# oxfordcontrol/COSMO.jl

Measured on AMD Instinct MI355X. Metric: ADMM iterations/sec (fp64) at fixed (n,m,nnz,cone), higher is better.
Workload: dtype f64

## Files before the change

cosmo.jl_amd/csrc/psd_polar.hip:

```cpp
#include "psd_internal.h"
#include "polar_tiles.h"
#include <math.h>
#include <stdlib.h>
#include <string.h>
#include <algorithm>
#include <mutex>

#define PK 16
#ifndef POLAR_PREFETCH_DEPTH
#define POLAR_PREFETCH_DEPTH 2
#endif
#define PLD 80
static_assert(PK == kPolarPanelK, "the planner's k panel");
static_assert(sizeof(QTile) == sizeof(int4), "the quadrant list is uploaded as the kernels' int4 array");

struct SkSync { unsigned ticket; unsigned timeout; unsigned pad[14]; unsigned flag[1]; };
struct PolarDev {
  int gate;
  int rounds;
  int verified;
  int unverified;
  int projections;
  int pad[3];
  real err_last, err_max;
};

static const real kPolarLift[3] = {3.8438259784376458, -2.5414431444903771, 0.42553478492344637};
#define POLAR_NFIN 5
static const real kPolarFinish[POLAR_NFIN][3] = {
    {3.4931704678738202, -2.370790022242379, 0.42240833954524776},
    {2.7077959763108326, -2.015093165601975, 0.45683257965863566},
    {1.9693651031668091, -1.3512768962961363, 0.3852630352029357},
    {1.875, -1.25, 0.375},
    {1.875, -1.25, 0.375}};
#define POLAR_RLIFT 3
#define POLAR_NFIN_LARGE (REAL_IS_FLOAT ? 4 : POLAR_NFIN)
#define POLAR_RLIFT_LARGE (REAL_IS_FLOAT ? 4 : POLAR_RLIFT)

#define POLAR_LIFT_CAP 18
struct PolarPlan {
  std::vector<PolarCone> cones;
  real* W = nullptr;
  real* parts = nullptr;
  real* nrm = nullptr;
  int k_lift = REAL_IS_FLOAT ? 5 : 9;
  bool klift_forced = false;
  int max_rounds = 2;
  int rescale = 1;
  int batch_occ = 3;
  real tol_factor = 8.0;
  PolarDev* dev = nullptr;
  PolarDev seen;
  long long launches[4] = {0, 0, 0, 0};
  int streamk = 0;
  real* sk_scratch = nullptr;
  SkSync* sk_sync = nullptr;
  int sk_gmax = 0;
  unsigned sk_base = 0, sk_epoch = 0;
  int products_last_large = 0, products_last_batch = 0;
  std::vector<BatchCone> bcones;
  BatchCone* d_bcones = nullptr;
  int4* d_btiles = nullptr;
  int nbtiles = 0, nbtiles96 = 0;
  int speculate = 0;
  int* gate_host = nullptr;
  int batch_wave = 0;
  int batch_ragged = 1;
  void* d_rtiles = nullptr;
  int nrtiles = 0;
  int dataflow = 0;
  void* d_df_tiles = nullptr;
  int* d_df_cone_nt = nullptr;
  unsigned* d_df_sync = nullptr;
  int df_xoff[9] = {0, 0, 0, 0, 0, 0, 0, 0, 0};
  int df_grid = 0;
  int df_pair = 3;
  int df_ntiles = 0;
  long long df_launches = 0, df_timed = 0;
  int df_nprod = 0;
  double df_seconds = 0.0;
  hipEvent_t df_ev[2] = {nullptr, nullptr};
  int df_ev_pending = 0;
  void* h_rtiles = nullptr;
  void* rep_host = nullptr;
  void* d_rtiles_rep = nullptr;
  int nrep = 0;
  long long repair_launch_tiles = 0, repair_trains = 0;
  double batch_flops_performed = 0.0, batch_flops_useful = 0.0;
  int batch_ts96 = 0;
  real* BW = nullptr;
  real* bparts = nullptr;
  real* bnrm = nullptr;
  int* bgate = nullptr;
  int adapt = 0;
  int compact_repair = 1;
  std::vector<LiftDepth> bdepth;
  int* d_lgate = nullptr;
  int* d_ubuf = nullptr;
  int* bgate_host = nullptr;
  int lgate_kmax = -1;
  long long depth_fail = 0, depth_down = 0, depth_proj = 0;
  int seen_proj_batch = 0;
  std::vector<LiftDepth> ldepth;
  int seen_proj_large = 0;
  double wprod_last = 0.0;
  bool adaptive() const { return adapt && !speculate && !klift_forced && k_lift <= POLAR_LIFT_CAP; }
};

extern "C" int32_t cosmo_hip_polar_schedule(int32_t k_lift, double* abc, int32_t* nsteps) {
  if (k_lift < 0 || k_lift > 64 || !nsteps) return COSMO_HIP_ERR_INVALID;
  *nsteps = k_lift + POLAR_NFIN;
  if (!abc) return COSMO_HIP_OK;
  for (int t = 0; t < k_lift; ++t) for (int q = 0; q < 3; ++q) abc[3 * t + q] = (double)kPolarLift[q];
  for (int t = 0; t < POLAR_NFIN; ++t) for (int q = 0; q < 3; ++q) abc[3 * (k_lift + t) + q] = (double)kPolarFinish[t][q];
  return COSMO_HIP_OK;
}

namespace {

__device__ __forceinline__ long long svec_index(int i, int j) { return (long long)j * (j + 1) / 2 + i; }


__device__ __forceinline__ real polar_read(const real* __restrict__ x, int kind, int d, int i, int j) {
  const real isq2 = 0.70710678118654752440;
  if (kind == COSMO_HIP_PSD_TRIANGLE) {
    const int a = i < j ? i : j, b = i < j ? j : i;
    const real t = x[svec_index(a, b)];
    return (a == b) ? t : isq2 * t;
  }
  if (kind == COSMO_HIP_PSD_SQUARE) {
    const int a = i < j ? i : j, b = i < j ? j : i;
    return (x[(long long)b * d + a] + x[(long long)a * d + b]) / R(2.0);
  }
  const int r = d / 2;
  const int bi = i >= r, bj = j >= r, ii = i - bi * r, jj = j - bj * r;
  const int a = ii < jj ? ii : jj, b = ii < jj ? jj : ii;
  if (bi == bj) { const real t = x[svec_index(a, b)]; return (a == b) ? t : isq2 * t; }
  if (ii == jj) return 0.0;
  real im = isq2 * x[(long long)r * (r + 1) / 2 + (long long)b * (b - 1) / 2 + a];
  if (ii > jj) im = -im;
  return (bi == 1) ? im : -im;
}
__device__ __forceinline__ void polar_write(real* __restrict__ x, int kind, int d, int i, int j, real v) {
  const real sq2 = 1.41421356237309504880;
  if (kind == COSMO_HIP_PSD_TRIANGLE) { x[svec_index(i, j)] = (i == j) ? v : sq2 * v; return; }
  if (kind == COSMO_HIP_PSD_SQUARE) { x[(long long)j * d + i] = v; x[(long long)i * d + j] = v; return; }
  const int r = d / 2;
  if (j < r) { x[svec_index(i, j)] = (i == j) ? v : sq2 * v; return; }
  if (i < r) { const int jj = j - r; if (i < jj) x[(long long)r * (r + 1) / 2 + (long long)jj * (jj - 1) / 2 + i] = sq2 * (-v); }
}

__global__ __launch_bounds__(COSMO_BS) void k_polar_populate(const Ctl* __restrict__ ctl, int guard, PolarCone cn, const real* __restrict__ s,
                                                             real* __restrict__ X, real* __restrict__ parts) {
  if (guard && ctl->halt) return;
  __shared__ real red[COSMO_BS / 64];
  const real* x = s + cn.off;
  const int d = cn.d, ld = cn.ld;
  real acc = 0.0;
  for (int j = blockIdx.x; j < ld; j += gridDim.x) {
    for (int i = threadIdx.x; i < ld; i += COSMO_BS) {
      real v = 0.0;
      if (i < d && j < d) { v = polar_read(x, cn.kind, d, i, j); acc += v * v; }
      X[(long long)j * ld + i] = v;
    }
  }
  acc = block_sum(acc, red);
  if (threadIdx.x == 0) parts[blockIdx.x] = acc;
}

__global__ __launch_bounds__(COSMO_BS) void k_polar_scale(const Ctl* __restrict__ ctl, int guard, long long n, int nparts, const real* __restrict__ parts,
                                                          const real* __restrict__ X, real* __restrict__ U, real* __restrict__ nrm_out) {
  if (guard && ctl->halt) return;
  __shared__ real red[COSMO_BS / 64];
  const real nf = sqrt(reduce_partials_sum(parts, nparts, red));
  const real inv = (nf > R(0.0)) ? R(2.0) / nf : R(0.0);
  if (blockIdx.x == 0 && threadIdx.x == 0) *nrm_out = nf;
// ... 1030 lines not shown

#define BPX 16
__global__ __launch_bounds__(COSMO_BS) void k_bpolar_populate(const Ctl* __restrict__ ctl, int guard, const BatchCone* __restrict__ cones,
                                                              const real* __restrict__ s, real* __restrict__ W, real* __restrict__ parts) {
  if (guard && ctl->halt) return;
  __shared__ real red[COSMO_BS / 64];
  const BatchCone cn = cones[blockIdx.y];
  const real* x = s + cn.off;
  real* X = W + cn.woff;
  const int d = cn.d, ld = cn.ld;
  real acc = 0.0;
  for (int j = blockIdx.x; j < ld; j += gridDim.x) {
    for (int i = threadIdx.x; i < ld; i += COSMO_BS) {
      real v = 0.0;
      if (i < d && j < d) { v = polar_read(x, cn.kind, d, i, j); acc += v * v; }
      X[(long long)j * ld + i] = v;
    }
  }
  acc = block_sum(acc, red);
  if (threadIdx.x == 0) parts[(size_t)blockIdx.y * 2 * BPX + blockIdx.x] = acc;
}
__global__ __launch_bounds__(COSMO_BS) void k_bpolar_scale(const Ctl* __restrict__ ctl, int guard, const BatchCone* __restrict__ cones,
                                                           const real* __restrict__ parts, real* __restrict__ W, real* __restrict__ bnrm,
                                                           const int* __restrict__ ubuf) {
  if (guard && ctl->halt) return;
  const BatchCone cn = cones[blockIdx.y];
  real nf2 = 0.0;
  for (int k = 0; k < BPX; ++k) nf2 += parts[(size_t)blockIdx.y * 2 * BPX + k];
  const real nf = sqrt(nf2);
  const real inv = (nf > R(0.0)) ? R(2.0) / nf : R(0.0);
  if (blockIdx.x == 0 && threadIdx.x == 0) bnrm[blockIdx.y] = nf;
  const long long n2 = (long long)cn.ld * cn.ld;
  const real* X = W + cn.woff;
  real* U = W + cn.woff + (ubuf ? ubuf[blockIdx.y] : 1) * n2;
  for (long long i = (long long)blockIdx.x * COSMO_BS + threadIdx.x; i < n2; i += (long long)gridDim.x * COSMO_BS) U[i] = X[i] * inv;
}
__global__ __launch_bounds__(COSMO_BS) void k_bpolar_finish(const Ctl* __restrict__ ctl, int guard, const BatchCone* __restrict__ cones,
                                                            real* __restrict__ W, int iu, real* __restrict__ s, real* __restrict__ parts) {
  if (guard && ctl->halt) return;
  __shared__ real red[COSMO_BS / 64];
  const BatchCone cn = cones[blockIdx.y];
  const long long n2 = (long long)cn.ld * cn.ld;
  const real* X = W + cn.woff;
  const real* U = W + cn.woff + iu * n2;
  const real* H = W + cn.woff + 3 * n2;
  real* x = s + cn.off;
  const int d = cn.d, ld = cn.ld;
  real tr = 0.0;
  for (int j = blockIdx.x; j < d; j += gridDim.x) {
    for (int i = threadIdx.x; i <= j; i += COSMO_BS) {
      const long long o = (long long)j * ld + i;
      const real v = (X[o] + H[o]) / R(2.0);
      polar_write(x, cn.kind, d, i, j, v);
      const real u = U[o];
      tr += (i == j) ? (u + u * u) : R(2.0) * u * u;
    }
  }
  tr = block_sum(tr, red);
  if (threadIdx.x == 0) parts[(size_t)blockIdx.y * 2 * BPX + BPX + blockIdx.x] = tr;
}
__global__ void k_bpolar_rank(const Ctl* __restrict__ ctl, int guard, int n, const BatchCone* __restrict__ cones, const real* __restrict__ parts,
                              int* __restrict__ rank) {
  if (guard && ctl->halt) return;
  const int c = blockIdx.x * blockDim.x + threadIdx.x;
  if (c >= n) return;
  real tr = 0.0;
  for (int k = 0; k < BPX; ++k) tr += parts[(size_t)c * 2 * BPX + BPX + k];
  rank[cones[c].idx] = (int)llround(tr / (cones[c].kind == COSMO_HIP_PSD_TRIANGLE_COMPLEX ? R(4.0) : R(2.0)));
}

__global__ __launch_bounds__(COSMO_BS) void k_bpolar_sumsq(const Ctl* __restrict__ ctl, int guard, const int* __restrict__ gate, const BatchCone* __restrict__ cones,
                                                           const real* __restrict__ W, int ig, real* __restrict__ vparts) {
  if (guard && ctl->halt) return;
  if (gate && !gate[blockIdx.y]) return;
  __shared__ real red[COSMO_BS / 64];
  const BatchCone cn = cones[blockIdx.y];
  const long long n2 = (long long)cn.ld * cn.ld;
  const real* G = W + cn.woff + ig * n2;
  real acc = 0.0;
  for (long long i = (long long)blockIdx.x * COSMO_BS + threadIdx.x; i < n2; i += (long long)gridDim.x * COSMO_BS) { const real v = G[i]; acc += v * v; }
  acc = block_sum(acc, red);
  if (threadIdx.x == 0) vparts[(size_t)blockIdx.y * BPX + blockIdx.x] = acc;
}
__global__ __launch_bounds__(COSMO_BS) void k_bpolar_decide(const Ctl* __restrict__ ctl, int guard, PolarDev* __restrict__ pd, int* __restrict__ bgate, int round,
                                                            int last, int n, const BatchCone* __restrict__ cones, const real* __restrict__ vparts,
                                                            const real* __restrict__ bnrm, real tol_factor) {
  if (guard && ctl->halt) return;
  if (round > 0 && !pd->gate) return;
  __shared__ real red[COSMO_BS / 64];
  real emax = 0.0, nfail = 0.0, nchk = 0.0;
  for (int c = threadIdx.x; c < n; c += COSMO_BS) {
    if (round > 0 && !bgate[c]) continue;
    real g2 = 0.0;
    for (int k = 0; k < BPX; ++k) g2 += vparts[(size_t)c * BPX + k];
    const real nf = bnrm[c];
    const real err = (nf > R(0.0)) ? R(0.5) * sqrt(g2) / nf : R(0.0);
    const bool ok = !(err > tol_factor * cones[c].d * PSD_EPS);
    bgate[c] = (!ok && !last) ? 1 : 0;
    nchk += 1.0;
    if (!ok) nfail += 1.0;
    emax = (err > emax || err != err) ? err : emax;
  }
  emax = block_max(emax, red);
  nfail = block_sum(nfail, red);
  nchk = block_sum(nchk, red);
  if (threadIdx.x != 0) return;
  pd->err_last = emax;
  if (emax > pd->err_max || emax != emax) pd->err_max = emax;
  if (round == 0) pd->projections += 1; else pd->rounds += 1;
  if (nfail == R(0.0)) { pd->verified += 1; pd->gate = 0; }
  else if (last) { pd->unverified += 1; pd->gate = 0; }
  else pd->gate = 1;
  (void)nchk;
}

}

void polar_plan_destroy(cosmo_hip_handle* h) {
  PolarPlan* q = static_cast<PolarPlan*>(h->psd_polar);
  if (!q) return;
  if (q->W) (void)hipFree(q->W);
  if (q->parts) (void)hipFree(q->parts);
  if (q->nrm) (void)hipFree(q->nrm);
  if (q->gate_host) (void)hipHostFree(q->gate_host);
  if (q->sk_scratch) (void)hipFree(q->sk_scratch);
  if (q->sk_sync) (void)hipFree(q->sk_sync);
  if (q->d_bcones) (void)hipFree(q->d_bcones);
  if (q->d_btiles) (void)hipFree(q->d_btiles);
  if (q->d_rtiles) (void)hipFree(q->d_rtiles);
  if (q->d_rtiles_rep) (void)hipFree(q->d_rtiles_rep);
  if (q->rep_host) (void)hipHostFree(q->rep_host);
  free(q->h_rtiles);
  if (q->BW) (void)hipFree(q->BW);
  if (q->bparts) (void)hipFree(q->bparts);
  if (q->bnrm) (void)hipFree(q->bnrm);
  if (q->bgate) (void)hipFree(q->bgate);
  if (q->d_lgate) (void)hipFree(q->d_lgate);
  if (q->d_ubuf) (void)hipFree(q->d_ubuf);
  if (q->bgate_host) (void)hipHostFree(q->bgate_host);
  if (q->d_df_tiles) (void)hipFree(q->d_df_tiles);
  if (q->d_df_cone_nt) (void)hipFree(q->d_df_cone_nt);
  if (q->d_df_sync) (void)hipFree(q->d_df_sync);
  if (q->df_ev[0]) { (void)hipEventDestroy(q->df_ev[0]); (void)hipEventDestroy(q->df_ev[1]); }
  if (q->dev) (void)hipFree(q->dev);
  delete q;
  h->psd_polar = nullptr;
}

bool polar_enabled(const cosmo_hip_handle* h) { return h->psd_polar != nullptr; }

struct PolarKnobs {
  int large_jacobi = -1, k_lift = -1, adapt = 0, compact_repair = 1, rescale = 1, speculate = -1, rounds = -1, patience = 3;
  int streamk = 0, ts = 0, sk = 0;
  long long skg = 0;
  int ts96 = 0, wave = 0, flat = 0, ragged = 1, paired = -1, sort = 1, dataflow = -1, dataflow_grid = -1, occ = -1;
};

static PolarKnobs polar_read_knobs() {
  PolarKnobs k;
  auto flag = [](const char* name, int dflt) { const char* e = getenv(name); return e ? (atoi(e) ? 1 : 0) : dflt; };
  auto within = [](const char* name, int lo, int hi, int dflt) { const char* e = getenv(name); const int v = e ? atoi(e) : dflt; return (v >= lo && v <= hi) ? v : dflt; };
  if (const char* e = getenv("COSMO_HIP_PSD_LARGE")) k.large_jacobi = (e[0] == 'j') ? 1 : 0;
  if (const char* e = getenv("COSMO_HIP_POLAR_KLIFT")) k.k_lift = std::min(40, std::max(0, atoi(e)));
  k.adapt = flag("COSMO_HIP_POLAR_ADAPT", k.adapt);
  if (const char* e = getenv("COSMO_HIP_POLAR_PATIENCE")) k.patience = std::max(1, atoi(e));
  k.compact_repair = flag("COSMO_HIP_POLAR_COMPACT_REPAIR", k.compact_repair);
  k.rescale = flag("COSMO_HIP_POLAR_RESCALE", k.rescale);
  k.speculate = flag("COSMO_HIP_POLAR_SPECULATE", k.speculate);
  if (const char* e = getenv("COSMO_HIP_POLAR_ROUNDS")) k.rounds = std::min(8, std::max(0, atoi(e)));
  k.streamk = flag("COSMO_HIP_POLAR_STREAMK", k.streamk);
  if (const char* e = getenv("COSMO_HIP_POLAR_TS")) k.ts = atoi(e);
  if (const char* e = getenv("COSMO_HIP_POLAR_SK")) k.sk = atoi(e);
  if (const char* e = getenv("COSMO_HIP_POLAR_SKG")) k.skg = atoll(e);
  k.ts96 = flag("COSMO_HIP_POLAR_BATCH_TS96", k.ts96);
  k.wave = flag("COSMO_HIP_POLAR_BATCH_WAVE", k.wave);
  k.flat = getenv("COSMO_HIP_POLAR_BATCH_FLAT") ? 1 : 0;
  k.ragged = flag("COSMO_HIP_POLAR_BATCH_RAGGED", k.ragged);
  k.sort = flag("COSMO_HIP_POLAR_BATCH_SORT", k.sort);
  k.occ = within("COSMO_HIP_POLAR_BATCH_OCC", 3, 4, k.occ);
  k.paired = within("COSMO_HIP_POLAR_PAIRED", 0, 3, k.paired);
  k.dataflow = flag("COSMO_HIP_POLAR_DATAFLOW", k.dataflow);
  k.dataflow_grid = within("COSMO_HIP_POLAR_DATAFLOW_GRID", 8, 8192, k.dataflow_grid);
  return k;
}

static void polar_set_func_attributes(const PolarPlan* q) {
  if (q->bcones.empty()) return;
  if (q->batch_ragged) {
    (void)hipFuncSetAttribute((const void*)k_polar_dataflow<4>, hipFuncAttributeMaxDynamicSharedMemorySize, GemmCfg<64>::SMEM);
    (void)hipFuncSetAttribute((const void*)k_polar_dataflow_pair<4>, hipFuncAttributeMaxDynamicSharedMemorySize, DF_PAIR_SMEM);
    (void)hipFuncSetAttribute((const void*)k_symm_gemm_batch_r<0, 3>, hipFuncAttributeMaxDynamicSharedMemorySize, GemmCfg<64>::SMEM);
    (void)hipFuncSetAttribute((const void*)k_symm_gemm_batch_r<1, 3>, hipFuncAttributeMaxDynamicSharedMemorySize, GemmCfg<64>::SMEM);
    (void)hipFuncSetAttribute((const void*)k_symm_gemm_batch_r<0, 4>, hipFuncAttributeMaxDynamicSharedMemorySize, GemmCfg<64>::SMEM);
    (void)hipFuncSetAttribute((const void*)k_symm_gemm_batch_r<1, 4>, hipFuncAttributeMaxDynamicSharedMemorySize, GemmCfg<64>::SMEM);
  }
  (void)hipFuncSetAttribute((const void*)k_symm_gemm_batch<0, 3, 64>, hipFuncAttributeMaxDynamicSharedMemorySize, GemmCfg<64>::SMEM);
  (void)hipFuncSetAttribute((const void*)k_symm_gemm_batch<1, 3, 64>, hipFuncAttributeMaxDynamicSharedMemorySize, GemmCfg<64>::SMEM);
  (void)hipFuncSetAttribute((const void*)k_symm_gemm_batch<0, 4, 64>, hipFuncAttributeMaxDynamicSharedMemorySize, GemmCfg<64>::SMEM);
  (void)hipFuncSetAttribute((const void*)k_symm_gemm_batch<1, 4, 64>, hipFuncAttributeMaxDynamicSharedMemorySize, GemmCfg<64>::SMEM);
  (void)hipFuncSetAttribute((const void*)k_symm_gemm_batch<0, 2, 96>, hipFuncAttributeMaxDynamicSharedMemorySize, GemmCfg<96>::SMEM);
  (void)hipFuncSetAttribute((const void*)k_symm_gemm_batch<1, 2, 96>, hipFuncAttributeMaxDynamicSharedMemorySize, GemmCfg<96>::SMEM);
}

template <class T>
static int32_t polar_upload(cosmo_hip_handle* h, T** dst, const void* src, size_t bytes) {
  HIPCHK(h, hipMalloc((void**)dst, bytes));
  HIPCHK(h, hipMemcpy(*dst, src, bytes, hipMemcpyHostToDevice));
  return COSMO_HIP_OK;
}

int32_t polar_plan_create(cosmo_hip_handle* h) {
  polar_plan_destroy(h);
  PsdPlan* p = h->psd;
  if (!p) return COSMO_HIP_OK;
  const PolarKnobs k = polar_read_knobs();
  std::vector<int> large_list, batch_list = p->polar_batch;
  const bool jac = k.large_jacobi >= 0 ? k.large_jacobi == 1 : h->psd_mode == 1;
  if (!jac) large_list = p->large;
  p->large_by_polar = !jac;
  for (int idx : p->cplx) { if (p->cones[idx].d > 256) large_list.push_back(idx); else batch_list.push_back(idx); }
  if (large_list.empty() && batch_list.empty()) return COSMO_HIP_OK;
  PolarPlan* q = new PolarPlan();
  h->psd_polar = q;
  q->klift_forced = k.k_lift >= 0;
  if (q->klift_forced) q->k_lift = k.k_lift;
  q->adapt = k.adapt; q->compact_repair = k.compact_repair; q->rescale = k.rescale; q->streamk = k.streamk;
  q->batch_ts96 = k.ts96; q->batch_wave = k.wave;
  q->speculate = k.speculate >= 0 ? k.speculate : (large_list.size() > 2 ? 1 : 0);
  if (k.rounds >= 0) q->max_rounds = k.rounds;
  q->batch_ragged = (k.ragged && !k.ts96 && !k.wave) ? 1 : 0;
  if (k.paired >= 0) q->df_pair = k.paired;
  PolarTileOpts o;
  o.ts96 = k.ts96; o.flat = k.flat; o.ragged = q->batch_ragged; o.pair = q->df_pair; o.sort = k.sort;
  o.streamk = k.streamk; o.ts = k.ts; o.sk = k.sk; o.skg = k.skg;
  HIPCHK(h, hipHostMalloc((void**)&q->gate_host, 8 * sizeof(int), hipHostMallocDefault));
  for (int i = 0; i < 8; ++i) q->gate_host[i] = 0;
  HIPCHK(h, hipMalloc((void**)&q->dev, sizeof(PolarDev)));
  HIPCHK(h, hipMemset(q->dev, 0, sizeof(PolarDev)));
  memset(&q->seen, 0, sizeof(PolarDev));
  if (!large_list.empty()) {
    long long woff = 0;
    for (int idx : large_list) {
      const PsdConeDev& c = p->cones[idx];
      PolarCone pc;
      pc.idx = idx; pc.off = c.off; pc.d = c.d; pc.kind = c.kind;
      polar_plan_large(o, pc);
      q->sk_gmax = std::max(q->sk_gmax, pc.skg);
      pc.woff = woff;
      woff += 4LL * pc.ld * pc.ld;
      q->cones.push_back(pc);
    }
    HIPCHK(h, hipMalloc((void**)&q->W, sizeof(real) * (size_t)woff));
    HIPCHK(h, hipMalloc((void**)&q->parts, sizeof(real) * 2 * COSMO_MAX_PARTIALS * q->cones.size()));
    HIPCHK(h, hipMalloc((void**)&q->nrm, sizeof(real) * q->cones.size()));
    if (q->sk_gmax > 0) {
      const size_t slot = (size_t)SKG_TS * SKG_TS;
      HIPCHK(h, hipMalloc((void**)&q->sk_scratch, sizeof(real) * slot * (size_t)q->sk_gmax));
      const size_t sb = sizeof(SkSync) + sizeof(unsigned) * (size_t)q->sk_gmax;
      HIPCHK(h, hipMalloc((void**)&q->sk_sync, sb));
      HIPCHK(h, hipMemset(q->sk_sync, 0, sb));
    }
  }
  if (!batch_list.empty()) {
    std::vector<PolarBatchIn> in;
    for (int idx : batch_list) { const PsdConeDev& c = p->cones[idx]; in.push_back(PolarBatchIn{c.d, c.off, c.kind, idx}); }
    PolarBatchPlan bp;
    if (const char* err = polar_plan_batch(in, o, bp)) return cosmo_fail(h, COSMO_HIP_ERR_INVALID, err);
    const size_t nb = bp.cones.size();
    q->bcones = bp.cones;
    q->nbtiles = bp.nbtiles; q->nbtiles96 = bp.nbtiles96;
    q->batch_flops_performed = bp.flops_performed; q->batch_flops_useful = bp.flops_useful;
    if (q->batch_ragged) {
      q->nrtiles = (int)bp.rtiles.size();
      q->df_ntiles = bp.df_ntiles;
      for (int x = 0; x <= kPolarXcds; ++x) q->df_xoff[x] = bp.xoff[x];
      if (q->df_pair) CHK(polar_upload(h, &q->d_df_tiles, bp.pairs.data(), sizeof(RPair) * bp.pairs.size()));
      else CHK(polar_upload(h, &q->d_df_tiles, bp.items.data(), sizeof(RTile) * bp.items.size()));
      CHK(polar_upload(h, &q->d_df_cone_nt, bp.cone_nt.data(), sizeof(int) * nb));
      HIPCHK(h, hipMalloc((void**)&q->d_df_sync, sizeof(unsigned) * (DF_SYNC_DONE + nb)));
      hipDeviceProp_t prop;
      HIPCHK(h, hipGetDeviceProperties(&prop, h->device));
      const int slots = std::max(1, prop.multiProcessorCount) * (q->df_pair ? 2 : 4);
      q->df_grid = k.dataflow_grid >= 0 ? k.dataflow_grid : std::max(1, prop.multiProcessorCount) * 4;
      int nmin = INT32_MAX;
      for (int x = 0; x < kPolarXcds; ++x) nmin = std::min(nmin, q->df_xoff[x + 1] - q->df_xoff[x]);
      q->dataflow = k.dataflow >= 0 ? k.dataflow : (nmin >= slots / kPolarXcds ? 1 : 0);
      const size_t rbytes = sizeof(RTile) * bp.rtiles.size();
      CHK(polar_upload(h, &q->d_rtiles, bp.rtiles.data(), rbytes));
      q->h_rtiles = malloc(rbytes);
      if (!q->h_rtiles) return cosmo_fail(h, COSMO_HIP_ERR_HIP, "out of host memory");
      memcpy(q->h_rtiles, bp.rtiles.data(), rbytes);
      HIPCHK(h, hipMalloc((void**)&q->d_rtiles_rep, rbytes));
      HIPCHK(h, hipHostMalloc((void**)&q->rep_host, rbytes));
    }
    HIPCHK(h, hipMalloc((void**)&q->BW, sizeof(real) * (size_t)bp.work));
    HIPCHK(h, hipMemset(q->BW, 0, sizeof(real) * (size_t)bp.work));
    CHK(polar_upload(h, &q->d_bcones, q->bcones.data(), sizeof(BatchCone) * nb));
    CHK(polar_upload(h, &q->d_btiles, bp.qtiles.data(), sizeof(QTile) * bp.qtiles.size()));
    HIPCHK(h, hipMalloc((void**)&q->bparts, sizeof(real) * 3 * BPX * nb));
    HIPCHK(h, hipMalloc((void**)&q->bnrm, sizeof(real) * nb));
    HIPCHK(h, hipMalloc((void**)&q->bgate, sizeof(int) * nb));
    HIPCHK(h, hipMemset(q->bgate, 0, sizeof(int) * nb));
    q->bdepth.assign(nb, LiftDepth{q->k_lift, 0, k.patience});
    HIPCHK(h, hipMalloc((void**)&q->d_lgate, sizeof(int) * nb * POLAR_LIFT_CAP));
    HIPCHK(h, hipMalloc((void**)&q->d_ubuf, sizeof(int) * nb));
    HIPCHK(h, hipHostMalloc((void**)&q->bgate_host, sizeof(int) * nb, hipHostMallocDefault));
    q->lgate_kmax = -1;
    q->batch_occ = k.occ >= 0 ? k.occ : (q->batch_ragged ? 4 : 3);
  }
  polar_set_func_attributes(q);
  return COSMO_HIP_OK;
}

bool polar_has_batch(const cosmo_hip_handle* h) { const PolarPlan* q = static_cast<const PolarPlan*>(h->psd_polar); return q && !q->bcones.empty(); }
bool polar_has_large(const cosmo_hip_handle* h) { const PolarPlan* q = static_cast<const PolarPlan*>(h->psd_polar); return q && !q->cones.empty(); }

template <int EPI>
static void launch_bgemm(PolarPlan* q, hipStream_t st, const Ctl* ctl, int guard, const int* gate, int ia, int ib, int icin, int ic, real alpha, real beta) {
  auto ragged = [&](int ntiles, const void* tiles) {
    const auto kern = q->batch_occ == 4 ? k_symm_gemm_batch_r<EPI, 4> : k_symm_gemm_batch_r<EPI, 3>;
    hipLaunchKernelGGL(kern, dim3(ntiles), dim3(256), GemmCfg<64>::SMEM, st, ctl, guard, gate, (const RTile*)tiles, q->d_bcones, q->BW, ia, ib, icin, ic, alpha, beta);
  };
  if (q->batch_ragged && q->nrep > 0) {
    ragged(q->nrep, q->d_rtiles_rep);
    q->repair_launch_tiles += q->nrep;
    return;
  }
  if (q->batch_ragged && q->nrtiles > 0) {
    ragged(q->nrtiles, q->d_rtiles);
    return;
  }
  if (q->nbtiles96 > 0)
    hipLaunchKernelGGL((k_symm_gemm_batch<EPI, 2, 96>), dim3(q->nbtiles96), dim3(256), GemmCfg<96>::SMEM, st, ctl, guard, gate, q->d_btiles + q->nbtiles,
                       q->d_bcones, q->BW, ia, ib, icin, ic, alpha, beta);
  if (q->nbtiles > 0 && q->batch_wave) {
    hipLaunchKernelGGL((k_symm_gemm_batch_w<EPI>), dim3(q->nbtiles), dim3(64), 0, st, ctl, guard, gate, q->d_btiles, q->d_bcones, q->BW, ia, ib, icin, ic, alpha, beta);
  } else if (q->nbtiles > 0) {
    const auto kern = q->batch_occ == 4 ? k_symm_gemm_batch<EPI, 4, 64> : k_symm_gemm_batch<EPI, 3, 64>;
    hipLaunchKernelGGL(kern, dim3(q->nbtiles), dim3(256), GemmCfg<64>::SMEM, st, ctl, guard, gate, q->d_btiles, q->d_bcones, q->BW, ia, ib, icin, ic, alpha, beta);
  }
}

int32_t polar_enqueue_project_batch(cosmo_hip_handle* h, real* s, int guard) {
  PolarPlan* q = static_cast<PolarPlan*>(h->psd_polar);
  PsdPlan* p = h->psd;
  hipStream_t st = h->stream;
  const int n = (int)q->bcones.size();
  real* vparts = q->bparts + (size_t)2 * BPX * n;
  const bool adapt = q->adaptive();
  int kmax = q->k_lift;
  if (adapt) {
    kmax = 0;
    for (int c = 0; c < n; ++c) kmax = std::max(kmax, q->bdepth[c].k);
    if (q->lgate_kmax != kmax) {
      std::vector<int> lg((size_t)std::max(kmax, 1) * n, 0), ub((size_t)n, 1);
      for (int c = 0; c < n; ++c) {
        const int t0 = kmax - q->bdepth[c].k;
        for (int t = t0; t < kmax; ++t) lg[(size_t)t * n + c] = 1;
        ub[(size_t)c] = (t0 & 1) ? 2 : 1;
      }
      HIPCHK(h, hipMemcpyAsync(q->d_lgate, lg.data(), sizeof(int) * lg.size(), hipMemcpyHostToDevice, st));
      HIPCHK(h, hipMemcpyAsync(q->d_ubuf, ub.data(), sizeof(int) * ub.size(), hipMemcpyHostToDevice, st));
      HIPCHK(h, hipStreamSynchronize(st));
      q->lgate_kmax = kmax;
    }
  }
  hipLaunchKernelGGL(k_bpolar_populate, dim3(BPX, n), dim3(COSMO_BS), 0, st, h->ctl, guard, q->d_bcones, s, q->BW, q->bparts);
  hipLaunchKernelGGL(k_bpolar_scale, dim3(BPX, n), dim3(COSMO_BS), 0, st, h->ctl, guard, q->d_bcones, q->bparts, q->BW, q->bnrm, adapt ? (const int*)q->d_ubuf : (const int*)nullptr);
  int iu = 1, iy = 2, products = 0;
  DfArgs dfa;
  bool df = q->dataflow && q->batch_ragged && q->nrtiles > 0 && !adapt && !h->profiling && 3 * (kmax + POLAR_NFIN) + 2 <= DF_MAX_PROD;
  dfa.nprod = 0;
  auto product = [&](int epi, const int* gate, int ia, int ib, int icin, int ic, real alpha, real beta) {
    if (df) { DfProd& pr = dfa.prod[dfa.nprod++]; pr.ia = ia; pr.ib = ib; pr.icin = icin; pr.ic = ic; pr.epi = epi; pr.pad = 0; pr.alpha = alpha; pr.beta = beta; return; }
    if (epi) launch_bgemm<1>(q, st, h->ctl, guard, gate, ia, ib, icin, ic, alpha, beta);
    else launch_bgemm<0>(q, st, h->ctl, guard, gate, ia, ib, icin, ic, alpha, beta);
  };
  auto flush_dataflow = [&]() -> int32_t {
    if (!df) return COSMO_HIP_OK;
    for (int x = 0; x < 9; ++x) dfa.xoff[x] = q->df_xoff[x];
    HIPCHK(h, hipMemsetAsync(q->d_df_sync, 0, sizeof(unsigned) * (DF_SYNC_DONE + q->bcones.size()), st));
    if (!q->df_ev[0]) { HIPCHK(h, hipEventCreate(&q->df_ev[0])); HIPCHK(h, hipEventCreate(&q->df_ev[1])); }
    if (q->df_ev_pending && hipEventQuery(q->df_ev[1]) == hipSuccess) {
      float ms = 0.f;
      if (hipEventElapsedTime(&ms, q->df_ev[0], q->df_ev[1]) == hipSuccess) { q->df_seconds += 1e-3 * (double)ms; q->df_timed += 1; }
      q->df_ev_pending = 0;
    }
    (void)hipGetLastError();
    const bool timed = !q->df_ev_pending;
    if (timed) HIPCHK(h, hipEventRecord(q->df_ev[0], st));
    if (q->df_pair)
      hipLaunchKernelGGL((k_polar_dataflow_pair<4>), dim3(q->df_grid), dim3(512), DF_PAIR_SMEM, st, h->ctl, guard, (const RPair*)q->d_df_tiles, (const int*)q->d_df_cone_nt,
                         q->d_df_sync, q->BW, dfa);
    else
      hipLaunchKernelGGL((k_polar_dataflow<4>), dim3(q->df_grid), dim3(256), GemmCfg<64>::SMEM, st, h->ctl, guard, (const RTile*)q->d_df_tiles, (const int*)q->d_df_cone_nt,
                         q->d_df_sync, q->BW, dfa);
    if (timed) { HIPCHK(h, hipEventRecord(q->df_ev[1], st)); q->df_ev_pending = 1; }
    q->df_launches += 1; q->df_nprod = dfa.nprod;
    df = false;
    return COSMO_HIP_OK;
  };
  auto step = [&](const real* co, const int* gate) {
    product(0, gate, iu, iu, iu, iy, 1.0, 0.0);
    product(1, gate, iy, iy, iy, 3, co[2], co[1]);
    product(1, gate, iu, 3, iu, iy, 1.0, co[0]);
    std::swap(iu, iy);
    products += 3; q->launches[3] += 3;
  };
  auto verify = [&](int round, const int* gate) -> int32_t {
    product(0, gate, iu, 0, 0, 3, 1.0, 0.0);
    product(1, gate, iu, 3, 0, iy, 1.0, -1.0);
    CHK(flush_dataflow());
    hipLaunchKernelGGL(k_bpolar_sumsq, dim3(BPX, n), dim3(COSMO_BS), 0, st, h->ctl, guard, gate, q->d_bcones, q->BW, iy, vparts);
    hipLaunchKernelGGL(k_bpolar_decide, dim3(1), dim3(COSMO_BS), 0, st, h->ctl, guard, q->dev, q->bgate, round, round == q->max_rounds ? 1 : 0, n, q->d_bcones,
                       vparts, q->bnrm, q->tol_factor);
    products += 2; q->launches[3] += 2;
    return COSMO_HIP_OK;
  };
  for (int t = 0; t < kmax; ++t) step(kPolarLift, adapt ? (const int*)(q->d_lgate + (size_t)t * n) : (const int*)nullptr);
  for (int t = 0; t < POLAR_NFIN; ++t) step(kPolarFinish[t], nullptr);
  CHK(verify(0, nullptr));
  q->products_last_batch = products;
  { double wsum = 0.0, w3 = 0.0;
    for (int c = 0; c < n; ++c) { const double d3 = (double)q->bcones[c].d * q->bcones[c].d * q->bcones[c].d; w3 += d3; wsum += d3 * (3.0 * ((adapt ? q->bdepth[c].k : kmax) + POLAR_NFIN) + 2.0); }
    q->wprod_last = w3 > 0.0 ? wsum / w3 : 0.0; }
  for (int r = 1; r <= q->max_rounds; ++r) {
    if (!q->speculate) {
      HIPCHK(h, hipMemcpyAsync(q->gate_host, &q->dev->gate, (adapt && r == 1 ? 5 : 1) * sizeof(int), hipMemcpyDeviceToHost, st));
      if (r == 1 && q->bgate_host) HIPCHK(h, hipMemcpyAsync(q->bgate_host, q->bgate, sizeof(int) * (size_t)n, hipMemcpyDeviceToHost, st));
      HIPCHK(h, hipStreamSynchronize(st));
      if (adapt && r == 1 && q->gate_host[4] != q->seen_proj_batch) {
        q->seen_proj_batch = q->gate_host[4];
        q->depth_proj += 1;
        bool changed = false;
        for (int c = 0; c < n; ++c) {
          if (*q->gate_host && q->bgate_host[c]) { q->depth_fail += 1; if (q->bdepth[c].fail(POLAR_LIFT_CAP)) changed = true; }
          else if (q->bdepth[c].pass(0)) { q->depth_down += 1; changed = true; }
        }
        if (changed) q->lgate_kmax = -1;
      }
      if (!*q->gate_host) break;
    }
    int rlift = POLAR_RLIFT;
    if (q->compact_repair && q->batch_ragged && q->h_rtiles && q->bgate_host && !q->speculate) {
      if (r == 1) {
        const RTile* all = (const RTile*)q->h_rtiles; RTile* dst = (RTile*)q->rep_host;
        int cnt = 0;
        for (int t = 0; t < q->nrtiles; ++t) if (all[t].cone >= 0 && q->bgate_host[all[t].cone]) dst[cnt++] = all[t];
        if (cnt > 0) {
          HIPCHK(h, hipMemcpyAsync(q->d_rtiles_rep, dst, sizeof(RTile) * (size_t)cnt, hipMemcpyHostToDevice, st));
          q->nrep = cnt; q->repair_trains += 1;
        }
        if (adapt) rlift = 1;
      }
    }
    for (int t = 0; t < rlift; ++t) step(kPolarLift, q->bgate);
    for (int t = 0; t < POLAR_NFIN; ++t) step(kPolarFinish[t], q->bgate);
    CHK(verify(r, q->bgate));
  }
  q->nrep = 0;
  hipLaunchKernelGGL(k_bpolar_finish, dim3(BPX, n), dim3(COSMO_BS), 0, st, h->ctl, guard, q->d_bcones, q->BW, iu, s, q->bparts);
  hipLaunchKernelGGL(k_bpolar_rank, dim3((n + 63) / 64), dim3(64), 0, st, h->ctl, guard, n, q->d_bcones, q->bparts, p->rank);
  HIPCHK(h, hipGetLastError());
  return COSMO_HIP_OK;
}

int32_t polar_enqueue_project(cosmo_hip_handle* h, real* s, int guard) {
  PolarPlan* q = static_cast<PolarPlan*>(h->psd_polar);
  PsdPlan* p = h->psd;
  hipStream_t st = h->stream;
  for (size_t ci = 0; ci < q->cones.size(); ++ci) {
    const PolarCone& cn = q->cones[ci];
    const long long n2 = (long long)cn.ld * cn.ld;
    real* X = q->W + cn.woff;
    real* U = X + n2;
    real* Y = U + n2;
    real* T = Y + n2;
    real* nparts = q->parts + 2 * COSMO_MAX_PARTIALS * ci;
    real* tparts = nparts + COSMO_MAX_PARTIALS;
    const int gpop = std::min(cn.ld, 1024);
    int products = 0;
    hipLaunchKernelGGL(k_polar_populate, dim3(gpop), dim3(COSMO_BS), 0, st, h->ctl, guard, cn, s, X, nparts);
    hipLaunchKernelGGL(k_polar_scale, dim3(1024), dim3(COSMO_BS), 0, st, h->ctl, guard, n2, gpop, nparts, X, U, q->nrm + ci);
    auto step = [&](const real* co, const int* gate) {
      symm_gemm(h, guard, gate, cn.ts, cn.sk, 0, U, U, nullptr, Y, cn.ld, 1.0, 0.0, cn.skg, cn.skc);
      symm_gemm(h, guard, gate, cn.ts, cn.sk, 1, Y, Y, Y, T, cn.ld, co[2], co[1], cn.skg, cn.skc);
      symm_gemm(h, guard, gate, cn.ts, cn.sk, 1, U, T, U, Y, cn.ld, 1.0, co[0], cn.skg, cn.skc);
      std::swap(U, Y);
      products += 3;
    };
    auto verify = [&](int round, const int* gate) {
      symm_gemm(h, guard, gate, cn.ts, cn.sk, 0, U, X, nullptr, T, cn.ld, 1.0, 0.0, cn.skg, cn.skc);
      symm_gemm(h, guard, gate, cn.ts, cn.sk, 1, U, T, X, Y, cn.ld, 1.0, -1.0, cn.skg, cn.skc);
      hipLaunchKernelGGL(k_polar_sumsq, dim3(1024), dim3(COSMO_BS), 0, st, h->ctl, guard, gate, n2, Y, nparts);
      hipLaunchKernelGGL(k_polar_decide, dim3(1), dim3(COSMO_BS), 0, st, h->ctl, guard, q->dev, round, round == q->max_rounds ? 1 : 0, 1024, nparts,
                         q->nrm + ci, q->tol_factor * cn.d * PSD_EPS);
      products += 2;
    };
    const bool adapt = q->adaptive();
    if (adapt && q->ldepth.size() != q->cones.size()) q->ldepth.assign(q->cones.size(), LiftDepth{q->k_lift, 0, 3});
    int k_main = adapt ? q->ldepth[ci].k : q->k_lift;
    if (q->rescale && k_main > 0) {
      symm_gemm(h, guard, nullptr, cn.ts, cn.sk, 0, U, U, nullptr, Y, cn.ld, 1.0, 0.0, cn.skg, cn.skc);
      hipLaunchKernelGGL(k_polar_sumsq, dim3(1024), dim3(COSMO_BS), 0, st, h->ctl, guard, (const int*)nullptr, n2, Y, nparts);
      hipLaunchKernelGGL(k_polar_rescale, dim3(1024), dim3(COSMO_BS), 0, st, h->ctl, guard, n2, 1024, nparts, U, Y);
      symm_gemm(h, guard, nullptr, cn.ts, cn.sk, 1, Y, Y, Y, T, cn.ld, kPolarLift[2], kPolarLift[1], cn.skg, cn.skc);
      symm_gemm(h, guard, nullptr, cn.ts, cn.sk, 1, U, T, U, Y, cn.ld, 1.0, kPolarLift[0], cn.skg, cn.skc);
      std::swap(U, Y);
      products += 3;
      k_main -= 1;
      if (cn.d >= 1024 && k_main > 1) k_main -= 1;
    }
    for (int t = 0; t < k_main; ++t) step(kPolarLift, nullptr);
    for (int t = 0; t < POLAR_NFIN_LARGE; ++t) step(kPolarFinish[t], nullptr);
    verify(0, nullptr);
    q->products_last_large = products;
    for (int r = 1; r <= q->max_rounds; ++r) {
      if (!q->speculate) {
        HIPCHK(h, hipMemcpyAsync(q->gate_host, &q->dev->gate, (adapt && r == 1 ? 5 : 1) * sizeof(int), hipMemcpyDeviceToHost, st));
        HIPCHK(h, hipStreamSynchronize(st));
        if (adapt && r == 1 && q->gate_host[4] != q->seen_proj_large) {
          q->seen_proj_large = q->gate_host[4];
          q->depth_proj += 1;
          if (*q->gate_host) { q->depth_fail += 1; q->ldepth[ci].fail(POLAR_LIFT_CAP); }
          else if (q->ldepth[ci].pass(2)) q->depth_down += 1;
        }
        if (!*q->gate_host) break;
      }
      for (int t = 0; t < POLAR_RLIFT_LARGE; ++t) step(kPolarLift, &q->dev->gate);
      for (int t = 0; t < POLAR_NFIN_LARGE; ++t) step(kPolarFinish[t], &q->dev->gate);
      verify(r, &q->dev->gate);
    }
    const int gfin = std::min(cn.d, 1024);
    hipLaunchKernelGGL(k_polar_finish, dim3(gfin), dim3(COSMO_BS), 0, st, h->ctl, guard, cn, X, T, U, s, tparts);
    hipLaunchKernelGGL(k_polar_rank, dim3(1), dim3(COSMO_BS), 0, st, h->ctl, guard, cn.d, gfin, tparts, p->rank + cn.idx, cn.kind);
  }
  HIPCHK(h, hipGetLastError());
  return COSMO_HIP_OK;
}

int32_t polar_adapt(cosmo_hip_handle* h) {
  PolarPlan* q = static_cast<PolarPlan*>(h->psd_polar);
  if (!q || !q->dev || h->comm || q->klift_forced) return COSMO_HIP_OK;
  if (q->adapt && !q->speculate) return COSMO_HIP_OK;
  PolarDev now;
// ... 181 lines not shown
```

Measured before the change: 377.3.

## Fuse batched polar entry, finish/rank and verify/decide passes with ticket counters

Adds fused kernels for the batched polar PSD projection. Entry uses a norm kernel plus a tiled, shared-memory transposed populate+scale. Finish and rank merge into one kernel that reduces the trace through a last-block ticket. The sum-of-squares pass merges with the single-block decide pass via per-cone and global atomic tickets, with the last arriving workgroup making the decision. The default passes=3 enables the new entry and finish_rank paths, while the fused verify stays off unless selected. The aim is fewer kernel launches and less global traffic per projection, at the cost of atomic ticket synchronisation and fence-ordering risk.

```diff
diff --git a/cosmo.jl_amd/csrc/psd_polar.hip b/cosmo.jl_amd/csrc/psd_polar.hip
--- a/cosmo.jl_amd/csrc/psd_polar.hip
+++ b/cosmo.jl_amd/csrc/psd_polar.hip
@@ -92,6 +92,8 @@
   real* bparts = nullptr;
   real* bnrm = nullptr;
   int* bgate = nullptr;
+  int passes = 3;
+  unsigned* d_pticket = nullptr;
   int adapt = 0;
   int compact_repair = 1;
   std::vector<LiftDepth> bdepth;
@@ -1288,12 +1290,8 @@
   acc = block_sum(acc, red);
   if (threadIdx.x == 0) vparts[(size_t)blockIdx.y * BPX + blockIdx.x] = acc;
 }
-__global__ __launch_bounds__(COSMO_BS) void k_bpolar_decide(const Ctl* __restrict__ ctl, int guard, PolarDev* __restrict__ pd, int* __restrict__ bgate, int round,
-                                                            int last, int n, const BatchCone* __restrict__ cones, const real* __restrict__ vparts,
-                                                            const real* __restrict__ bnrm, real tol_factor) {
-  if (guard && ctl->halt) return;
-  if (round > 0 && !pd->gate) return;
-  __shared__ real red[COSMO_BS / 64];
+__device__ __forceinline__ void bpolar_decide_body(PolarDev* __restrict__ pd, int* bgate, int round, int last, int n, const BatchCone* __restrict__ cones,
+                                                   const real* vparts, const real* __restrict__ bnrm, real tol_factor, real* red) {
   real emax = 0.0, nfail = 0.0, nchk = 0.0;
   for (int c = threadIdx.x; c < n; c += COSMO_BS) {
     if (round > 0 && !bgate[c]) continue;
@@ -1318,6 +1316,168 @@
   else if (last) { pd->unverified += 1; pd->gate = 0; }
   else pd->gate = 1;
   (void)nchk;
+}
+__global__ __launch_bounds__(COSMO_BS) void k_bpolar_decide(const Ctl* __restrict__ ctl, int guard, PolarDev* __restrict__ pd, int* __restrict__ bgate, int round,
+                                                            int last, int n, const BatchCone* __restrict__ cones, const real* __restrict__ vparts,
+                                                            const real* __restrict__ bnrm, real tol_factor) {
+  if (guard && ctl->halt) return;
+  if (round > 0 && !pd->gate) return;
+  __shared__ real red[COSMO_BS / 64];
+  bpolar_decide_body(pd, bgate, round, last, n, cones, vparts, bnrm, tol_factor, red);
+}
+
+#define BP_LD(p) __hip_atomic_load((p), __ATOMIC_RELAXED, __HIP_MEMORY_SCOPE_AGENT)
+#define BP_ST(p, v) __hip_atomic_store((p), (v), __ATOMIC_RELAXED, __HIP_MEMORY_SCOPE_AGENT)
+__device__ __forceinline__ unsigned bp_ticket(unsigned* cnt) {
+  asm volatile("s_waitcnt vmcnt(0)" ::: "memory");
+  return __hip_atomic_fetch_add(cnt, 1u, __ATOMIC_RELAXED, __HIP_MEMORY_SCOPE_AGENT);
+}
+
+__global__ __launch_bounds__(COSMO_BS) void k_bpolar_norm(const Ctl* __restrict__ ctl, int guard, const BatchCone* __restrict__ cones,
+                                                          const real* __restrict__ s, real* __restrict__ parts) {
+  if (guard && ctl->halt) return;
+  __shared__ real red[COSMO_BS / 64];
+  const BatchCone cn = cones[blockIdx.y];
+  const real* x = s + cn.off;
+  const int d = cn.d;
+  real acc = 0.0;
+  for (int j = blockIdx.x; j < d; j += BPX) {
+    for (int i = threadIdx.x; i < d; i += COSMO_BS) { const real v = polar_read(x, cn.kind, d, i, j); acc += v * v; }
+  }
+  acc = block_sum(acc, red);
+  if (threadIdx.x == 0) parts[(size_t)blockIdx.y * 2 * BPX + blockIdx.x] = acc;
+}
+#define BP_TP 65
+__global__ __launch_bounds__(COSMO_BS) void k_bpolar_entry(const Ctl* __restrict__ ctl, int guard, const BatchCone* __restrict__ cones, const real* __restrict__ s,
+                                                           const real* __restrict__ parts, real* __restrict__ W, real* __restrict__ bnrm,
+                                                           const int* __restrict__ ubuf) {
+  if (guard && ctl->halt) return;
+  __shared__ real T[64 * BP_TP];
+  const BatchCone cn = cones[blockIdx.y];
+  real nf2 = 0.0;
+  for (int k = 0; k < BPX; ++k) nf2 += parts[(size_t)blockIdx.y * 2 * BPX + k];
+  const real nf = sqrt(nf2);
+  const real inv = (nf > R(0.0)) ? R(2.0) / nf : R(0.0);
+  if (blockIdx.x == 0 && threadIdx.x == 0) bnrm[blockIdx.y] = nf;
+  const real* x = s + cn.off;
+  const int d = cn.d, ld = cn.ld;
+  const long long n2 = (long long)ld * ld;
+  real* X = W + cn.woff;
+  real* U = W + cn.woff + (ubuf ? ubuf[blockIdx.y] : 1) * n2;
+  const int nt = (ld + 63) >> 6, w = threadIdx.x >> 6, lane = threadIdx.x & 63;
+  for (int t = (blockIdx.x + blockIdx.y) % BPX; t < nt * (nt + 1) / 2; t += BPX) {
+    int J = 0, I = t;
+    while (I > J) { I -= J + 1; ++J; }
+    const int i0 = I << 6, j0 = J << 6;
+    for (int c = w; c < 64; c += COSMO_BS / 64) {
+      const int i = i0 + lane, j = j0 + c;
+      T[c * BP_TP + lane] = (i <= j && j < d) ? polar_read(x, cn.kind, d, i, j) : R(0.0);
+    }
+    __syncthreads();
+    for (int c = w; c < 64; c += COSMO_BS / 64) {
+      const int i = i0 + lane, j = j0 + c;
+      if (i < ld && j < ld) {
+        const real v = (i <= j) ? T[c * BP_TP + lane] : T[lane * BP_TP + c];
+        const long long o = (long long)j * ld + i;
+        X[o] = v;
+        U[o] = v * inv;
+      }
+      const int im = j0 + lane, jm = i0 + c;
+      if (I != J && im < ld && jm < ld) {
+        const real v = T[lane * BP_TP + c];
+        const long long o = (long long)jm * ld + im;
+        X[o] = v;
+        U[o] = v * inv;
+      }
+    }
+    __syncthreads();
+  }
+}
+__global__ __launch_bounds__(COSMO_BS) void k_bpolar_finish_rank(const Ctl* __restrict__ ctl, int guard, const BatchCone* __restrict__ cones,
+                                                                 const real* __restrict__ W, int iu, real* __restrict__ s, real* parts,
+                                                                 unsigned* __restrict__ ticket, int* __restrict__ rank) {
+  if (guard && ctl->halt) return;
+  __shared__ real red[COSMO_BS / 64];
+  const BatchCone cn = cones[blockIdx.y];
+  const long long n2 = (long long)cn.ld * cn.ld;
+  const real* X = W + cn.woff;
+  const real* U = W + cn.woff + iu * n2;
+  const real* H = W + cn.woff + 3 * n2;
+  real* x = s + cn.off;
+  const int d = cn.d, ld = cn.ld;
+  real tr = 0.0;
+  if (d <= COSMO_BS) {
+    const int i = threadIdx.x;
+    for (int jb = blockIdx.x; jb < d; jb += 4 * BPX) {
+      real u[4];
+#pragma unroll
+      for (int k = 0; k < 4; ++k) { const int j = jb + k * BPX; u[k] = (j < d && i <= j) ? U[(long long)j * ld + i] : R(0.0); }
+#pragma unroll
+      for (int k = 0; k < 4; ++k) { const int j = jb + k * BPX; if (j < d && i <= j) tr += (i == j) ? (u[k] + u[k] * u[k]) : R(2.0) * u[k] * u[k]; }
+    }
+  } else {
+    for (int j = blockIdx.x; j < d; j += BPX) {
+      for (int i = threadIdx.x; i <= j; i += COSMO_BS) {
+        const real u = U[(long long)j * ld + i];
+        tr += (i == j) ? (u + u * u) : R(2.0) * u * u;
+      }
+    }
+  }
+  const int nseg = (d + 63) >> 6;
+  for (int u = blockIdx.x * (COSMO_BS / 64) + (threadIdx.x >> 6); u < d * nseg; u += BPX * (COSMO_BS / 64)) {
+    const int j = u / nseg, i = ((u - j * nseg) << 6) + (threadIdx.x & 63);
+    if (i <= j) {
+      const long long o = (long long)j * ld + i;
+      polar_write(x, cn.kind, d, i, j, (X[o] + H[o]) / R(2.0));
+    }
+  }
+  tr = block_sum(tr, red);
+  if (threadIdx.x != 0) return;
+  real* tp = parts + (size_t)blockIdx.y * 2 * BPX + BPX;
+  BP_ST(tp + blockIdx.x, tr);
+  if (bp_ticket(ticket + blockIdx.y) != BPX - 1) return;
+  real t[BPX];
+#pragma unroll
+  for (int k = 0; k < BPX; ++k) t[k] = BP_LD(tp + k);
+  real sum = 0.0;
+#pragma unroll
+  for (int k = 0; k < BPX; ++k) sum += t[k];
+  rank[cn.idx] = (int)llround(sum / (cn.kind == COSMO_HIP_PSD_TRIANGLE_COMPLEX ? R(4.0) : R(2.0)));
+  BP_ST(ticket + blockIdx.y, 0u);
+}
+__global__ __launch_bounds__(COSMO_BS) void k_bpolar_verify(const Ctl* __restrict__ ctl, int guard, PolarDev* __restrict__ pd, int* bgate, int round, int last,
+                                                            int n, const int* gate, const BatchCone* __restrict__ cones, const real* __restrict__ W, int ig,
+                                                            real* vparts, const real* __restrict__ bnrm, real tol_factor, unsigned* __restrict__ ticket) {
+  if (guard && ctl->halt) return;
+  __shared__ real red[COSMO_BS / 64];
+  __shared__ unsigned s_last;
+  const bool skip = gate && !gate[blockIdx.y];
+  real acc = 0.0;
+  if (!skip) {
+    const BatchCone cn = cones[blockIdx.y];
+    const long long n2 = (long long)cn.ld * cn.ld;
+    const real* G = W + cn.woff + ig * n2;
+    for (long long i = (long long)blockIdx.x * COSMO_BS + threadIdx.x; i < n2; i += (long long)gridDim.x * COSMO_BS) { const real v = G[i]; acc += v * v; }
+    acc = block_sum(acc, red);
+  }
+  if (threadIdx.x == 0) {
+    if (!skip) BP_ST(vparts + (size_t)blockIdx.y * BPX + blockIdx.x, acc);
+    unsigned lastwg = 0u;
+    if (bp_ticket(ticket + blockIdx.y) == BPX - 1) {
+      BP_ST(ticket + blockIdx.y, 0u);
+      lastwg = __hip_atomic_fetch_add(ticket + gridDim.y, 1u, __ATOMIC_RELAXED, __HIP_MEMORY_SCOPE_AGENT) == gridDim.y - 1 ? 1u : 0u;
+      if (lastwg) {
+        __builtin_amdgcn_fence(__ATOMIC_ACQUIRE, "agent");
+        asm volatile("s_waitcnt vmcnt(0)" ::: "memory");
+      }
+    }
+    s_last = lastwg;
+  }
+  __syncthreads();
+  if (!s_last) return;
+  if (threadIdx.x == 0) BP_ST(ticket + gridDim.y, 0u);
+  if (round > 0 && !pd->gate) return;
+  bpolar_decide_body(pd, bgate, round, last, n, cones, vparts, bnrm, tol_factor, red);
 }
 
 }
@@ -1341,6 +1501,7 @@
   if (q->bparts) (void)hipFree(q->bparts);
   if (q->bnrm) (void)hipFree(q->bnrm);
   if (q->bgate) (void)hipFree(q->bgate);
+  if (q->d_pticket) (void)hipFree(q->d_pticket);
   if (q->d_lgate) (void)hipFree(q->d_lgate);
   if (q->d_ubuf) (void)hipFree(q->d_ubuf);
   if (q->bgate_host) (void)hipHostFree(q->bgate_host);
@@ -1359,7 +1520,7 @@
   int large_jacobi = -1, k_lift = -1, adapt = 0, compact_repair = 1, rescale = 1, speculate = -1, rounds = -1, patience = 3;
   int streamk = 0, ts = 0, sk = 0;
   long long skg = 0;
-  int ts96 = 0, wave = 0, flat = 0, ragged = 1, paired = -1, sort = 1, dataflow = -1, dataflow_grid = -1, occ = -1;
+  int ts96 = 0, wave = 0, flat = 0, ragged = 1, paired = -1, sort = 1, dataflow = -1, dataflow_grid = -1, occ = -1, passes = -1;
 };
 
 static PolarKnobs polar_read_knobs() {
@@ -1387,6 +1548,7 @@
   k.paired = within("COSMO_HIP_POLAR_PAIRED", 0, 3, k.paired);
   k.dataflow = flag("COSMO_HIP_POLAR_DATAFLOW", k.dataflow);
   k.dataflow_grid = within("COSMO_HIP_POLAR_DATAFLOW_GRID", 8, 8192, k.dataflow_grid);
+  k.passes = within("COSMO_HIP_POLAR_PASSES", 0, 7, k.passes);
   return k;
 }
 
@@ -1507,6 +1669,9 @@
     HIPCHK(h, hipMalloc((void**)&q->bnrm, sizeof(real) * nb));
     HIPCHK(h, hipMalloc((void**)&q->bgate, sizeof(int) * nb));
     HIPCHK(h, hipMemset(q->bgate, 0, sizeof(int) * nb));
+    if (k.passes >= 0) q->passes = k.passes;
+    HIPCHK(h, hipMalloc((void**)&q->d_pticket, sizeof(unsigned) * (nb + 1)));
+    HIPCHK(h, hipMemset(q->d_pticket, 0, sizeof(unsigned) * (nb + 1)));
     q->bdepth.assign(nb, LiftDepth{q->k_lift, 0, k.patience});
     HIPCHK(h, hipMalloc((void**)&q->d_lgate, sizeof(int) * nb * POLAR_LIFT_CAP));
     HIPCHK(h, hipMalloc((void**)&q->d_ubuf, sizeof(int) * nb));
@@ -1571,8 +1736,14 @@
       q->lgate_kmax = kmax;
     }
   }
-  hipLaunchKernelGGL(k_bpolar_populate, dim3(BPX, n), dim3(COSMO_BS), 0, st, h->ctl, guard, q->d_bcones, s, q->BW, q->bparts);
-  hipLaunchKernelGGL(k_bpolar_scale, dim3(BPX, n), dim3(COSMO_BS), 0, st, h->ctl, guard, q->d_bcones, q->bparts, q->BW, q->bnrm, adapt ? (const int*)q->d_ubuf : (const int*)nullptr);
+  const int* ubuf = adapt ? (const int*)q->d_ubuf : (const int*)nullptr;
+  if (q->passes & 1) {
+    hipLaunchKernelGGL(k_bpolar_norm, dim3(BPX, n), dim3(COSMO_BS), 0, st, h->ctl, guard, q->d_bcones, s, q->bparts);
+    hipLaunchKernelGGL(k_bpolar_entry, dim3(BPX, n), dim3(COSMO_BS), 0, st, h->ctl, guard, q->d_bcones, s, q->bparts, q->BW, q->bnrm, ubuf);
+  } else {
+    hipLaunchKernelGGL(k_bpolar_populate, dim3(BPX, n), dim3(COSMO_BS), 0, st, h->ctl, guard, q->d_bcones, s, q->BW, q->bparts);
+    hipLaunchKernelGGL(k_bpolar_scale, dim3(BPX, n), dim3(COSMO_BS), 0, st, h->ctl, guard, q->d_bcones, q->bparts, q->BW, q->bnrm, ubuf);
+  }
   int iu = 1, iy = 2, products = 0;
   DfArgs dfa;
   bool df = q->dataflow && q->batch_ragged && q->nrtiles > 0 && !adapt && !h->profiling && 3 * (kmax + POLAR_NFIN) + 2 <= DF_MAX_PROD;
@@ -1617,9 +1788,14 @@
     product(0, gate, iu, 0, 0, 3, 1.0, 0.0);
     product(1, gate, iu, 3, 0, iy, 1.0, -1.0);
     CHK(flush_dataflow());
-    hipLaunchKernelGGL(k_bpolar_sumsq, dim3(BPX, n), dim3(COSMO_BS), 0, st, h->ctl, guard, gate, q->d_bcones, q->BW, iy, vparts);
-    hipLaunchKernelGGL(k_bpolar_decide, dim3(1), dim3(COSMO_BS), 0, st, h->ctl, guard, q->dev, q->bgate, round, round == q->max_rounds ? 1 : 0, n, q->d_bcones,
-                       vparts, q->bnrm, q->tol_factor);
+    if (q->passes & 4) {
+      hipLaunchKernelGGL(k_bpolar_verify, dim3(BPX, n), dim3(COSMO_BS), 0, st, h->ctl, guard, q->dev, q->bgate, round, round == q->max_rounds ? 1 : 0, n, gate,
+                         q->d_bcones, q->BW, iy, vparts, q->bnrm, q->tol_factor, q->d_pticket);
+    } else {
+      hipLaunchKernelGGL(k_bpolar_sumsq, dim3(BPX, n), dim3(COSMO_BS), 0, st, h->ctl, guard, gate, q->d_bcones, q->BW, iy, vparts);
+      hipLaunchKernelGGL(k_bpolar_decide, dim3(1), dim3(COSMO_BS), 0, st, h->ctl, guard, q->dev, q->bgate, round, round == q->max_rounds ? 1 : 0, n, q->d_bcones,
+                         vparts, q->bnrm, q->tol_factor);
+    }
     products += 2; q->launches[3] += 2;
     return COSMO_HIP_OK;
   };
@@ -1665,8 +1841,12 @@
     CHK(verify(r, q->bgate));
   }
   q->nrep = 0;
-  hipLaunchKernelGGL(k_bpolar_finish, dim3(BPX, n), dim3(COSMO_BS), 0, st, h->ctl, guard, q->d_bcones, q->BW, iu, s, q->bparts);
-  hipLaunchKernelGGL(k_bpolar_rank, dim3((n + 63) / 64), dim3(64), 0, st, h->ctl, guard, n, q->d_bcones, q->bparts, p->rank);
+  if (q->passes & 2) {
+    hipLaunchKernelGGL(k_bpolar_finish_rank, dim3(BPX, n), dim3(COSMO_BS), 0, st, h->ctl, guard, q->d_bcones, q->BW, iu, s, q->bparts, q->d_pticket, p->rank);
+  } else {
+    hipLaunchKernelGGL(k_bpolar_finish, dim3(BPX, n), dim3(COSMO_BS), 0, st, h->ctl, guard, q->d_bcones, q->BW, iu, s, q->bparts);
+    hipLaunchKernelGGL(k_bpolar_rank, dim3((n + 63) / 64), dim3(64), 0, st, h->ctl, guard, n, q->d_bcones, q->bparts, p->rank);
+  }
   HIPCHK(h, hipGetLastError());
   return COSMO_HIP_OK;
 }
```

Result: no change. 374.0 (-0.9%).
